# radhofan/Fairify

Hardware: AMD Instinct MI355X
Metric: % partitions verified + partitions/sec on AC suite at 1/2/4/8 MI355X (higher is better)
Workload: dtype fp32

## Files before the change

fairify_amd/csrc/symbolic.hip:

```cpp
#include <hip/hip_runtime.h>

#include <tuple>

#include "args.h"
#include "launch.h"

#define FA_SYM_MAXC 48

struct SymCfg {
  int nc;
  int cdim[FA_SYM_MAXC];
  unsigned long long fold;
  int w_lds[FA_MAX_LAYERS];
  int b_lds[FA_MAX_LAYERS];
  int lds_floats;
  int stage_off;
  int stage_floats;
};

using SymShapeAny = FaShapeAny;
template <int... D>
using SymShape = FaShape<D...>;

template <class S>
struct SymLay {
  __host__ __device__ static constexpr int tiles(int n) { return (n + 15) >> 4; }
  __host__ __device__ static constexpr int w(int l) {
    int off = 0;
    for (int i = 0; i < l; ++i) off += tiles(S::dim(i)) * tiles(S::dim(i + 1)) * 256;
    return off;
  }
  __host__ __device__ static constexpr int b(int l) {
    int off = w(S::L);
    for (int i = 0; i < l; ++i) off += S::dim(i + 1);
    return off;
  }
  __host__ __device__ static constexpr int noff(int l) {
    int off = 0;
    for (int i = 0; i < l; ++i) off += S::dim(i + 1);
    return off;
  }
  static constexpr int STAGE = (b(S::L) + 3) & ~3;
  static constexpr int LDS = STAGE + FA_SYM_MAXC;
};

struct SymBox {
  const BoundArgs* a;
  int node, v, n0;
  __device__ __forceinline__ float lo(int d) const {
    float x = a->lo[(size_t)node * n0 + d];
    if (a->V > 0)
      for (int k = 0; k < a->npa; ++k)
        if (a->pa_idx[k] == d) x = a->values[v * a->npa + k];
    return x;
  }
  __device__ __forceinline__ float hi(int d) const {
    float x = a->hi[(size_t)node * n0 + d];
    if (a->V > 0)
      for (int k = 0; k < a->npa; ++k)
        if (a->pa_idx[k] == d) x = a->values[v * a->npa + k];
    return x;
  }
};

__device__ __forceinline__ int fa_trot(int rho) { return rho >> 3; }

template <int NT, int PG = 1>
struct SymSlab {
  static constexpr int TS = 16 * NT + 4;
  static constexpr int TILE1 = 2 * 16 * TS;
  static constexpr int TILE = 2 * TILE1;
  static constexpr int BOX = 3 * FA_SYM_MAXC;
  static constexpr int BOXTAB = PG > 1 ? 2 * PG * 32 : 0;
  static constexpr int FLOATS = (TILE + 2 * PG * BOX + BOXTAB + 3) & ~3;
};

template <bool PAIR, int TM>
struct SymForm {
  static constexpr bool CR = !PAIR && TM >= 2;
};

__device__ __forceinline__ void fa_pq_to_ul(const f32x4& P, const f32x4& Q, int fc, float gg, f32x4& U,
                                            f32x4& L) {
  const float sl = (fc == 1 || fc == 3) ? 2.f * gg : 0.f;
#pragma unroll
  for (int i = 0; i < 4; ++i) {
    const float q = Q[i], e = sl * fabsf(q);
    U[i] = (P[i] + q) + e;
    L[i] = (P[i] - q) - e;
  }
}

template <int NT, bool PAIR, int PG = 1, bool CR = false, class S = SymShapeAny, bool MASK = true>
__device__ __forceinline__ bool fa_sym_epilogue(const NetDesc& net, const BoundArgs& a, const SymCfg& cfg,
                                                const float* smem, float* T, const float* bxv_in, const int* cdim_s,
                                                int l, int r_in, int node_in, int r2, int node2, bool v2, int lane,
                                                int jt0, const f32x4 (&U)[2][NT],
                                                const f32x4 (&Lq)[2][NT], float (&nu)[2][NT][4],
                                                float (&nlo)[2][NT][4]) {
  constexpr int TS = SymSlab<NT>::TS;
  constexpr bool CS = S::L > 0;
  constexpr bool CL = CS && PG == 1;
  const int col = lane & 15, grp = lane >> 4;
  const int n_out = CS ? S::dim(l + 1) : net.dims[l + 1];
  const float* sb = smem + (CL ? SymLay<S>::b(l) : cfg.b_lds[l]);
  const bool last = CS ? l == S::L - 1 : l == net.n_layers - 1;
  const float gg = net.g_gemm[l];
  const float gc = net.g_conc;
  const float gi = net.g_one;
  const float unit = net.unit;
  const float gnext = last ? 0.f : (CR ? net.g_fwd[l + 1] : net.g_gemm[l + 1]);
  const int noff = CL ? SymLay<S>::noff(l) : net.neuron_off[l];
  const int nc = cfg.nc;
  const int n0 = CS ? S::dim(0) : net.dims[0];
  const int tsub = lane >> 5;
  const bool second = PAIR && tsub;
  constexpr int PS = 16 / PG;
  const int gbox = PG > 1 ? col / PS : 0;
  const int bidx = tsub * PG + gbox;
  const int r = PG > 1 ? r_in + bidx : (second ? r2 : r_in);
  const int node = PG > 1 ? (a.V > 0 ? r / a.V : r) : (second ? node2 : node_in);
  const float* bxv = bxv_in + (PG > 1 ? bidx : (second ? 1 : 0)) * SymSlab<NT, PG>::BOX;
  const int jt = PAIR ? jt0 : jt0 + tsub;
  const int n_out_t = n_out;
  const bool nl_act = PG > 1 ? r < a.R : (16 * jt < n_out_t && (!second || v2));
  const int ob = (lane >> 4) & 1;
  float* Trow = T + tsub * SymSlab<NT>::TILE1 + (ob * 16 + col) * TS + fa_trot(ob * 16 + col);
#pragma unroll
    for (int u = 0; u < 2; ++u)
#pragma unroll
      for (int ct = 0; ct < NT; ++ct)
#pragma unroll
        for (int i = 0; i < 4; ++i) {
          const int ru = 4 * grp + i, rl = 16 + 4 * grp + i;
          T[u * SymSlab<NT>::TILE1 + ru * TS + fa_trot(ru) + ct * 16 + col] = U[u][ct][i];
          T[u * SymSlab<NT>::TILE1 + rl * TS + fa_trot(rl) + ct * 16 + col] = Lq[u][ct][i];
        }
    __builtin_amdgcn_wave_barrier();
    const int j = PG > 1 ? col - gbox * PS : 16 * jt + col;
    const bool jv = j < n_out;
    float v[16 * NT];
#pragma unroll
    for (int c = 0; c < 16 * NT; ++c) v[c] = Trow[c];
    const float braw = sb[PG > 1 ? col : min(j, n_out - 1)];
    const float b = jv ? braw : 0.f;
    float s1 = 0.f, s2 = 0.f, mg = 0.f;
#pragma unroll
    for (int c = 4; c < 16 * NT; ++c) {
      const float av = fabsf(v[c]);
      s1 = fmaf(v[c], bxv[c], s1);
      s2 = fmaf(av, bxv[FA_SYM_MAXC + c], s2);
      mg = fmaf(av, bxv[2 * FA_SYM_MAXC + c], mg);
    }
    float mn = s1 - s2, mx = s1 + s2;
    const float cr = v[0];
    float er = v[1], ivr = v[2], ier = v[3];
    const float sgn = ob ? -1.f : 1.f;
    er *= sgn;
    ier *= sgn;
    const float c0 = cr + b;
    const float mgc = mg;
    mn += c0; mx += c0; mg += fabsf(c0);
    const float iv = ivr + b;
    const float eI = ier * (1.f + 2.f * gg) + gg * fabsf(b);
    const float e = er * (1.f + 2.f * gg) + gg * fabsf(b);
    float bound;
    if (ob == 0) bound = fminf(iv + gi * fabsf(iv) + eI, mx + gc * mg + e);
    else bound = fmaxf(iv - gi * fabsf(iv) - eI, mn - gc * mg - e);
    const float other = __shfl_xor(bound, 16, 64);
    const float ub = ob == 0 ? bound : other;
    const float lb = ob == 0 ? other : bound;
    if (nl_act && jv && a.layer_lb) {
      if (ob == 0) a.layer_ub[(size_t)r * net.n_neurons + noff + j] = ub;
      else a.layer_lb[(size_t)r * net.n_neurons + noff + j] = lb;
    }
    if (last) {
      if (PG > 1) {
        if (nl_act && j == 0) {
          float* Cf = ob == 0 ? a.Uc : a.Lc;
          if (ob == 0) {
            a.out_ub[r] = ub; a.U0[r] = c0; a.Ue[r] = e;
          } else {
            a.out_lb[r] = lb; a.L0[r] = c0; a.Le[r] = e;
          }
          for (int d = 0; d < n0; ++d)
            if ((cfg.fold >> d) & 1ull) Cf[(size_t)r * n0 + d] = 0.f;
          for (int c = 0; c < nc; ++c) Cf[(size_t)r * n0 + cdim_s[c]] = Trow[4 + c];
        }
      } else if (nl_act && jt == 0) {
        if (col == 0) {
          if (ob == 0) {
            a.out_ub[r] = ub; a.U0[r] = c0; a.Ue[r] = e;
          } else {
            a.out_lb[r] = lb; a.L0[r] = c0; a.Le[r] = e;
          }
        }
        float* Cf = (ob == 0 ? a.Uc : a.Lc) + (size_t)r * n0;
        const float* row0 = T + tsub * SymSlab<NT>::TILE1 + (ob * 16) * TS + fa_trot(ob * 16) + 4;
        const unsigned long long fold = cfg.fold;
        for (int d = col; d < n0; d += 16) {
          const bool folded = (fold >> d) & 1ull;
          const int c = d - __popcll(fold & ((1ull << d) - 1ull));
          const float x = row0[folded ? 0 : c];
          Cf[d] = folded ? 0.f : x;
        }
      }
      return false;
    }
    bool forced = false, fact = false;
    if (MASK && nl_act && jv) {
      if (a.dead_in) forced = a.dead_in[(size_t)r * net.n_hidden + noff + j] != 0;
      else if (a.dead_part) forced = a.dead_part[(size_t)a.node_part[node] * net.n_hidden + noff + j] != 0;
      if (a.phase_in) {
        const int8_t ph = a.phase_in[(size_t)r * net.n_hidden + noff + j];
        forced = forced || ph < 0;
        fact = ph > 0;
        if (ob == 0 && a.infeas && ((ph < 0 && lb > 0.f) || (ph > 0 && ub < 0.f))) a.infeas[r] = 1;
      }
    }
    const bool isdead = ub <= 0.f;
    const bool isact = lb >= 0.f;
    if (MASK && nl_act && ob == 0 && jv && a.dead_out) a.dead_out[(size_t)r * net.n_hidden + noff + j] = isdead ? 1 : 0;
    const bool zero = isdead || forced || !jv;
    const float aa = mn - gc * mg + e;
    const float bb = mx + gc * mg + e;
    const bool chord = !zero && !isact && !fact && aa < 0.f;
    const float sc = (bb / (bb - aa)) * (1.f + 4.f * unit);
    const float shift = e - aa;
    const float cc = c0 * sc + sc * shift;
    const float sU = zero ? 0.f : (chord ? sc : 1.f);
    const float cU = zero ? 0.f : (chord ? cc : c0);
    const float mU = zero ? 0.f : (chord ? sc * mgc * (1.f + 8.f * unit) + fabsf(cc) : mg);
    const float eU = zero ? 0.f : (chord ? 4.f * unit * sc * (mg + fabsf(shift)) : e);
    const float aL = mn - gc * mg - e;
    const float bL = mx + gc * mg - e;
    const bool lam1 = !zero && (isact || ((bL > 0.f) && (bL > -aL)));
    const bool up = ob == 0;
    const float ivn = zero ? 0.f : fmaxf(up ? ub : lb, 0.f);
    const float s = up ? sU : (lam1 ? 1.f : 0.f);
    const float cnew = up ? cU : (lam1 ? c0 : 0.f);
    const float en = up ? eU : (lam1 ? e : 0.f);
    const float mgn = up ? mU : (lam1 ? mg : 0.f);
    const float mg_b = CR ? mgn + __shfl_xor(mgn, 16, 64) : mgn;
    const float iv_b = CR ? fmaxf(ivn, __shfl_xor(ivn, 16, 64)) : ivn;
    v[0] = cnew;
    v[1] = sgn * (en + gnext * mg_b);
    v[2] = ivn;
    v[3] = sgn * (gnext * iv_b);
#pragma unroll
    for (int c = 4; c < 16 * NT; ++c) v[c] *= s;
    if (nl_act) {
#pragma unroll
      for (int c = 0; c < 16 * NT; ++c) Trow[c] = v[c];
    }
    __builtin_amdgcn_wave_barrier();
#pragma unroll
    for (int u = 0; u < 2; ++u)
#pragma unroll
      for (int ct = 0; ct < NT; ++ct)
#pragma unroll
        for (int i = 0; i < 4; ++i) {
          const int ru = 4 * grp + i, rl = 16 + 4 * grp + i;
          const float xu = T[u * SymSlab<NT>::TILE1 + ru * TS + fa_trot(ru) + ct * 16 + col];
          const float xl = T[u * SymSlab<NT>::TILE1 + rl * TS + fa_trot(rl) + ct * 16 + col];
          nu[u][ct][i] = CR ? 0.5f * (xu + xl) : xu;
          nlo[u][ct][i] = CR ? 0.5f * (xu - xl) : xl;
        }
    __builtin_amdgcn_wave_barrier();
    return true;
}

template <int NT, int TM, bool PAIR, int PG = 1, class S = SymShapeAny, bool MASK = true>
__device__ __forceinline__ void fa_sym_layer(const NetDesc& net, const BoundArgs& a, const SymCfg& cfg,
                                             const float* smem, float* T, const float* bxv, const int* cdim_s,
                                             int l, int r, int node, int r2, int node2, bool v2, int lane,
                                             const float (&B)[NT][PAIR ? 2 : TM][2][4],
                                             float (&A)[NT][PAIR ? 2 : TM][2][4]) {
  constexpr int TMS = PAIR ? 2 : TM;
  constexpr bool CR = SymForm<PAIR, TM>::CR;
  constexpr int TS = SymSlab<NT>::TS;
  constexpr bool CS = S::L > 0;
  constexpr bool CL = CS && PG == 1;
  const int col = lane & 15, grp = lane >> 4;
  const int n_in = CS ? S::dim(l) : net.dims[l], n_out = CS ? S::dim(l + 1) : net.dims[l + 1];
  const int tin = (n_in + 15) >> 4, tout = (n_out + 15) >> 4;
  const float* sw = smem + (CL ? SymLay<S>::w(l) : cfg.w_lds[l]);
  const bool last = CS ? l == S::L - 1 : l == net.n_layers - 1;
  const float gg = net.g_gemm[l];
  const int nc = cfg.nc;
  const int n0 = CS ? S::dim(0) : net.dims[0];
#ifndef FA_SYM_TIMING_NO_EPILOGUE
  if (PG > 1 && l == 0) {
    const float* boxtab = bxv + 2 * PG * SymSlab<NT, PG>::BOX;
    const float g0 = net.g_gemm[0];
    const int n0v = n0;
    f32x4 U[2][NT], Lq[2][NT];
#pragma unroll
    for (int u = 0; u < 2; ++u) {
#pragma unroll
      for (int ct = 0; ct < NT; ++ct) U[u][ct] = Lq[u][ct] = f32x4{0.f, 0.f, 0.f, 0.f};
#pragma unroll
      for (int g = 0; g < PG; ++g) {
        const float* bt = boxtab + (u * PG + g) * 32;
        const float4 w4 = reinterpret_cast<const float4*>(sw)[g * 64 + lane];
        const float wv[4] = {w4.x, w4.y, w4.z, w4.w};
#pragma unroll
        for (int i = 0; i < 4; ++i) {
          const int k = 4 * grp + i;
          const bool kv = k < n0v;
          const float xl = kv ? bt[k] : 0.f, xh = kv ? bt[16 + k] : 0.f;
          const bool folded = kv && ((cfg.fold >> k) & 1ull);
          const float m = fmaxf(fabsf(xl), fabsf(xh));
          const float wp = fmaxf(wv[i], 0.f), wn = fminf(wv[i], 0.f);
#pragma unroll
          for (int ct = 0; ct < NT; ++ct) {
            const int c = ct * 16 + col;
            float vu = 0.f, vl = 0.f;
            if (kv) {
              if (c >= 4) {
                vu = vl = (!folded && c - 4 < nc && cdim_s[c - 4] == k) ? 1.f : 0.f;
              } else if (c == 0) {
                vu = vl = folded ? xl : 0.f;
              } else if (c == 1) {
                vu = g0 * m; vl = -vu;
              } else if (c == 2) {
                vu = xh; vl = xl;
              } else {
                vu = g0 * fabsf(xh); vl = -(g0 * fabsf(xl));
              }
            }
            U[u][ct] = fa_mfma4(wp, vu, U[u][ct]);
            Lq[u][ct] = fa_mfma4(wp, vl, Lq[u][ct]);
            U[u][ct] = fa_mfma4(wn, vl, U[u][ct]);
            Lq[u][ct] = fa_mfma4(wn, vu, Lq[u][ct]);
          }
        }
      }
    }
    float nu[2][NT][4], nlo[2][NT][4];
    if (!fa_sym_epilogue<NT, PAIR, PG, CR, S, MASK>(net, a, cfg, smem, T, bxv, cdim_s, l, r, node, r2, node2, v2, lane, 0, U, Lq,
                                       nu, nlo))
      return;
#pragma unroll
    for (int u = 0; u < 2; ++u)
#pragma unroll
      for (int ct = 0; ct < NT; ++ct)
#pragma unroll
        for (int i = 0; i < 4; ++i) {
          A[ct][u][0][i] = nu[u][ct][i];
          A[ct][u][1][i] = nlo[u][ct][i];
        }
    return;
  }
  if (PG == 1 && last && n_out == 1) {
    constexpr int NB = PAIR ? 2 : 1;
    float su[NB][NT], sl[NB][NT];
#pragma unroll
    for (int bi = 0; bi < NB; ++bi)
#pragma unroll
      for (int ct = 0; ct < NT; ++ct) su[bi][ct] = sl[bi][ct] = 0.f;
#pragma unroll
    for (int t = 0; t < TM; ++t) {
      if (t >= tin) break;
      const float4 w4 = reinterpret_cast<const float4*>(sw)[t * 64 + grp * 16];
      const float wv[4] = {w4.x, w4.y, w4.z, w4.w};
#pragma unroll
      for (int i = 0; i < 4; ++i) {
        const float wp = fmaxf(wv[i], 0.f), wn = fminf(wv[i], 0.f);
#pragma unroll
        for (int bi = 0; bi < NB; ++bi)
#pragma unroll
          for (int ct = 0; ct < NT; ++ct) {
            const int bt = PAIR ? bi : t;
            if (CR) {
              su[bi][ct] = fmaf(wv[i], B[ct][bt][0][i], su[bi][ct]);
              sl[bi][ct] = fmaf(fabsf(wv[i]), B[ct][bt][1][i], sl[bi][ct]);
            } else {
              su[bi][ct] = fmaf(wp, B[ct][bt][0][i], fmaf(wn, B[ct][bt][1][i], su[bi][ct]));
              sl[bi][ct] = fmaf(wp, B[ct][bt][1][i], fmaf(wn, B[ct][bt][0][i], sl[bi][ct]));
            }
          }
      }
    }
    f32x4 U[2][NT], Lq[2][NT];
#pragma unroll
    for (int ct = 0; ct < NT; ++ct) U[1][ct] = Lq[1][ct] = f32x4{0.f, 0.f, 0.f, 0.f};
#pragma unroll
    for (int bi = 0; bi < NB; ++bi)
#pragma unroll
      for (int ct = 0; ct < NT; ++ct) {
        float xu = su[bi][ct], xl = sl[bi][ct];
        xu += __shfl_xor(xu, 16, 64);
        xl += __shfl_xor(xl, 16, 64);
        xu += __shfl_xor(xu, 32, 64);
        xl += __shfl_xor(xl, 32, 64);
        U[bi][ct] = f32x4{grp == 0 ? xu : 0.f, 0.f, 0.f, 0.f};
        Lq[bi][ct] = f32x4{grp == 0 ? xl : 0.f, 0.f, 0.f, 0.f};
        if (CR) fa_pq_to_ul(f32x4(U[bi][ct]), f32x4(Lq[bi][ct]), ct * 16 + col, gg, U[bi][ct], Lq[bi][ct]);
      }
    float nu[2][NT][4], nlo[2][NT][4];
    fa_sym_epilogue<NT, PAIR, PG, CR, S, MASK>(net, a, cfg, smem, T, bxv, cdim_s, l, r, node, r2, node2, v2, lane, 0, U, Lq,
                                  nu, nlo);
    return;
  }
#endif
#pragma unroll
  for (int jt0 = 0; jt0 < TM; jt0 += 2) {
    if (jt0 >= tout) break;
    f32x4 U[2][NT], Lq[2][NT];
#pragma unroll
    for (int u = 0; u < 2; ++u) {
      const int jt = jt0 + u;
#pragma unroll
      for (int ct = 0; ct < NT; ++ct) {
        U[u][ct] = f32x4{0.f, 0.f, 0.f, 0.f};
        Lq[u][ct] = f32x4{0.f, 0.f, 0.f, 0.f};
      }
      if (PAIR ? (jt0 > 0) : (jt >= tout || jt >= TM)) continue;
      const float4* wq = reinterpret_cast<const float4*>(sw) + (size_t)(PAIR ? 0 : jt) * tin * 64 + lane;
#pragma unroll
      for (int t = 0; t < TM; ++t) {
        if (t >= tin) break;
        const float4 w4 = wq[t * 64];
        const float wv[4] = {w4.x, w4.y, w4.z, w4.w};
#pragma unroll
        for (int i = 0; i < 4; ++i) {
          const float wp = fmaxf(wv[i], 0.f), wn = fminf(wv[i], 0.f);
#pragma unroll
          for (int ct = 0; ct < NT; ++ct) {
            const int bt = PAIR ? u : t;
            const float bu = B[ct][bt][0][i], bl = B[ct][bt][1][i];
            if (CR) {
              U[u][ct] = fa_mfma4(wv[i], bu, U[u][ct]);
              Lq[u][ct] = fa_mfma4(fabsf(wv[i]), bl, Lq[u][ct]);
            } else {
              U[u][ct] = fa_mfma4(wp, bu, U[u][ct]);
              Lq[u][ct] = fa_mfma4(wp, bl, Lq[u][ct]);
              U[u][ct] = fa_mfma4(wn, bl, U[u][ct]);
              Lq[u][ct] = fa_mfma4(wn, bu, Lq[u][ct]);
            }
          }
        }
      }
      if (CR) {
#pragma unroll
        for (int ct = 0; ct < NT; ++ct)
          fa_pq_to_ul(f32x4(U[u][ct]), f32x4(Lq[u][ct]), ct * 16 + col, gg, U[u][ct], Lq[u][ct]);
      }
    }
    float nu[2][NT][4], nlo[2][NT][4];
#ifdef FA_SYM_TIMING_NO_EPILOGUE
#pragma unroll
    for (int u = 0; u < 2; ++u)
#pragma unroll
      for (int ct = 0; ct < NT; ++ct)
#pragma unroll
        for (int i = 0; i < 4; ++i) {
          nu[u][ct][i] = U[u][ct][i] * 1e-3f;
          nlo[u][ct][i] = Lq[u][ct][i] * 1e-3f;
        }
    if (l == net.n_layers - 1) {
      if (lane == 0) a.out_lb[r] = nu[0][0][0] + nlo[0][0][1];
      continue;
    }
#else
    if (!fa_sym_epilogue<NT, PAIR, PG, CR, S, MASK>(net, a, cfg, smem, T, bxv, cdim_s, l, r, node, r2, node2, v2, lane, jt0, U,
                                       Lq, nu, nlo))
      continue;
#endif
#pragma unroll
    for (int u = 0; u < 2; ++u) {
      if (jt0 + u >= TMS) break;
#pragma unroll
      for (int ct = 0; ct < NT; ++ct)
#pragma unroll
        for (int i = 0; i < 4; ++i) {
          A[ct][jt0 + u][0][i] = nu[u][ct][i];
          A[ct][jt0 + u][1][i] = nlo[u][ct][i];
        }
    }
  }
}

#ifndef FA_SYM_WPE7
#define FA_SYM_WPE7 2
#endif
#ifndef FA_SYM_WPE4
#define FA_SYM_WPE4 2
#endif
#define FA_SYM_WAVES_PER_EU(NT, TM, PAIR) \
  ((PAIR) ? 3 : ((TM) == 2 ? 3 : ((TM) == 4 ? FA_SYM_WPE4 : ((TM) == 7 ? FA_SYM_WPE7 : 1))))

template <int NT, int TM, bool PAIR, int PG, class S, bool MASK, int... LS>
__device__ __forceinline__ void fa_sym_layers_c(std::integer_sequence<int, LS...>, const NetDesc& net,
                                                const BoundArgs& a, const SymCfg& cfg, const float* smem, float* T,
                                                const float* bxv, const int* cdim_s, int r, int node, int r2,
                                                int node2, bool v2, int lane, float (&XA)[NT][PAIR ? 2 : TM][2][4],
                                                float (&XB)[NT][PAIR ? 2 : TM][2][4]) {
  ((LS & 1 ? fa_sym_layer<NT, TM, PAIR, PG, S, MASK>(net, a, cfg, smem, T, bxv, cdim_s, LS, r, node, r2, node2, v2,
                                                     lane, XB, XA)
           : fa_sym_layer<NT, TM, PAIR, PG, S, MASK>(net, a, cfg, smem, T, bxv, cdim_s, LS, r, node, r2, node2, v2,
                                                     lane, XA, XB)),
   ...);
}

#ifndef FA_SYM_BIG_THREADS
#define FA_SYM_BIG_THREADS 512
#endif
#define FA_SYM_THREADS(TM) ((TM) == 7 ? FA_SYM_BIG_THREADS : FA_THREADS)

#ifndef FA_SYM_PREFETCH
#define FA_SYM_PREFETCH 1
#endif

template <int NT, int TM, bool PAIR, class S>
struct SymTune {
  static constexpr int THREADS = FA_SYM_THREADS(TM);
  static constexpr int WPE = FA_SYM_WAVES_PER_EU(NT, TM, PAIR);
};
#define FA_SYM_TUNE(NT, TM, THREADS_, WPE_, ...)            \
  template <>                                                \
  struct SymTune<NT, TM, false, FaShape<__VA_ARGS__>> {      \
    static constexpr int THREADS = THREADS_;                 \
    static constexpr int WPE = WPE_;                         \
  };
FA_SYM_TUNE(1, 7, 256, 3, 13, 100, 1)

__device__ __forceinline__ void fa_sym_box_values(float l0, float h0, float* bv, int lane) {
  float mid = 0.5f * (l0 + h0), rad = 0.5f * (h0 - l0), mm = fmaxf(fabsf(l0), fabsf(h0));
  const bool lattice = l0 == rintf(l0) && h0 == rintf(h0) && fabsf(l0) < 4194304.f && fabsf(h0) < 4194304.f;
  if (!lattice) {
    rad = nextafterf(fmaxf(h0 - mid, mid - l0), INFINITY);
    mm = nextafterf(fabsf(mid) + rad, INFINITY);
  }
  bv[lane] = mid;
  bv[FA_SYM_MAXC + lane] = rad;
  bv[2 * FA_SYM_MAXC + lane] = mm;
}

template <int NT, bool CR, int TMS>
__device__ __forceinline__ void fa_sym_operand0(float xl, float xh, bool kv, bool folded, int k, float g0,
                                                const int (&role)[NT], const int (&cdm)[NT],
                                                float (&XA)[NT][TMS][2][4], int t, int i) {
  const float m = fmaxf(fabsf(xl), fabsf(xh));
#pragma unroll
  for (int ct = 0; ct < NT; ++ct) {
    float vu = 0.f, vl = 0.f;
    if (kv) {
      switch (role[ct]) {
        case 0: vu = (!folded && cdm[ct] == k) ? 1.f : 0.f; vl = CR ? 0.f : vu; break;
        case 1: vu = folded ? xl : 0.f; vl = CR ? 0.f : vu; break;
        case 2: vu = CR ? 0.f : g0 * m; vl = CR ? g0 * m : -vu; break;
        case 3:
          vu = CR ? 0.5f * (xh + xl) : xh;
          vl = CR ? 0.5f * (xh - xl) : xl;
          break;
        case 4:
          vu = CR ? 0.5f * g0 * (fabsf(xh) - fabsf(xl)) : g0 * fabsf(xh);
          vl = CR ? 0.5f * g0 * (fabsf(xh) + fabsf(xl)) : -(g0 * fabsf(xl));
          break;
        default: break;
      }
    }
    XA[ct][t][0][i] = vu;
    XA[ct][t][1][i] = vl;
  }
}

template <int NT, int TM, bool PAIR, int PG, class S, bool MASK>
__device__ __forceinline__ void fa_sym_rows(const NetDesc& net, const BoundArgs& a, const SymCfg& cfg, float* smem,
                                            const int* cdim_s, int lds_floats) {
  constexpr int THREADS = SymTune<NT, TM, PAIR, S>::THREADS;
  constexpr bool CR = SymForm<PAIR, TM>::CR;
  constexpr int TMS = PAIR ? 2 : TM;
  const int tid = threadIdx.x;
  const int lane = tid & 63;
  const int grp = lane >> 4;
  const int wave = tid >> 6;
  const int nw = THREADS / 64;
  const int n0 = S::L > 0 ? S::dim(0) : net.dims[0];
  const int nc = cfg.nc;
  const float g0 = net.g_gemm[0];
  float* T = smem + lds_floats + wave * SymSlab<NT, PG>::FLOATS;
  float* bxv = T + SymSlab<NT>::TILE;
  const int tin0 = (n0 + 15) >> 4;
  int role[NT], cdm[NT];
#pragma unroll
  for (int ct = 0; ct < NT; ++ct) {
    const int c = ct * 16 + (lane & 15);
    role[ct] = c == 0 ? 1 : c == 1 ? 2 : c == 2 ? 3 : c == 3 ? 4 : (c - 4 < nc ? 0 : 5);
    cdm[ct] = (role[ct] == 0) ? cdim_s[c - 4] : -1;
  }
  constexpr int RPW = PAIR ? 2 * PG : 1;
  if constexpr (!PAIR && S::L > 0 && FA_SYM_PREFETCH) {
    float* btab = bxv + SymSlab<NT>::BOX;
    static_assert(SymSlab<NT>::BOX >= 128, "box table in the second box's slot");
    static_assert(S::dim(0) <= 64, "lane d carries input dim d");
    const int V = a.V, R = a.R;
    int pslot = -1;
    if (V > 0)
      for (int k = 0; k < a.npa; ++k)
        if (a.pa_idx[k] == lane) pslot = k;
    const int dl = min(lane, n0 - 1);
    const int stride = gridDim.x * nw;
    const bool filt = a.skip_status != nullptr;
    auto node_of = [&](int rr) { return V > 0 ? rr / V : rr; };
    auto fetch = [&](int rr, int node, float& blo, float& bhi) {
      blo = a.lo[(size_t)node * n0 + dl];
      bhi = a.hi[(size_t)node * n0 + dl];
      if (pslot >= 0) blo = bhi = a.values[(rr - node * V) * a.npa + pslot];
    };
    int r = __builtin_amdgcn_readfirstlane(blockIdx.x * nw + wave);
    float blo = 0.f, bhi = 0.f;
    int st = 3, part1 = 0;
    int node = 0;
    if (r < R) {
      node = node_of(r);
      fetch(r, node, blo, bhi);
      if (filt) st = a.skip_status[a.skip_part[node]];
      if (filt && r + stride < R) part1 = a.skip_part[node_of(r + stride)];
    }
    for (; r < R; r += stride) {
      const int rn = r + stride;
      float nlo = 0.f, nhi = 0.f;
      int nst = 3, part2 = 0, nnode = 0;
      if (rn < R) {
        nnode = node_of(rn);
        fetch(rn, nnode, nlo, nhi);
        if (filt) nst = a.skip_status[part1];
        if (filt && rn + stride < R) part2 = a.skip_part[node_of(rn + stride)];
      }
      if (st == 3 || st == 4) {
        btab[lane] = blo;
        btab[64 + lane] = bhi;
        __builtin_amdgcn_wave_barrier();
        if (lane < FA_SYM_MAXC) {
          const int d = (lane >= 4 && lane - 4 < nc) ? cdim_s[lane - 4] : -1;
          fa_sym_box_values(d >= 0 ? btab[max(d, 0)] : 0.f, d >= 0 ? btab[64 + max(d, 0)] : 0.f, bxv, lane);
        }
        float XA[NT][TMS][2][4], XB[NT][TMS][2][4];
#pragma unroll
        for (int t = 0; t < TMS; ++t) {
          if (t >= tin0) break;
          const float4 l4 = reinterpret_cast<const float4*>(btab)[(4 * t + grp) & 15];
          const float4 h4 = reinterpret_cast<const float4*>(btab + 64)[(4 * t + grp) & 15];
          const float xl4[4] = {l4.x, l4.y, l4.z, l4.w}, xh4[4] = {h4.x, h4.y, h4.z, h4.w};
#pragma unroll
          for (int i = 0; i < 4; ++i) {
            const int k = 16 * t + 4 * grp + i;
            const bool kv = k < n0;
            const float xl = kv ? xl4[i] : 0.f, xh = kv ? xh4[i] : 0.f;
            fa_sym_operand0<NT, CR>(xl, xh, kv, kv && ((cfg.fold >> k) & 1ull), k, g0, role, cdm, XA, t, i);
          }
        }
        __builtin_amdgcn_wave_barrier();
        fa_sym_layers_c<NT, TM, PAIR, PG, S, MASK>(std::make_integer_sequence<int, S::L>{}, net, a, cfg, smem, T, bxv,
                                                   cdim_s, r, node, r, node, false, lane, XA, XB);
        __builtin_amdgcn_wave_barrier();
      }
      blo = nlo;
      bhi = nhi;
      st = nst;
      part1 = part2;
      node = nnode;
    }
    return;
  }
  for (int r0 = (blockIdx.x * nw + wave) * RPW; r0 < a.R; r0 += gridDim.x * nw * RPW) {
    const int r = __builtin_amdgcn_readfirstlane(r0);
    const bool v2 = PAIR && r + 1 < a.R;
    const int rb = v2 ? r + 1 : r;
    if (a.skip_status) {
      bool any = false;
#pragma unroll
      for (int bi = 0; bi < RPW; ++bi) {
        const int rr = min(r + bi, a.R - 1);
        const int8_t s1 = a.skip_status[a.skip_part[a.V > 0 ? rr / a.V : rr]];
        any = any || s1 == 3 || s1 == 4;
      }
      if (!any) continue;
    }
    SymBox bxs[RPW];
#pragma unroll
    for (int bi = 0; bi < RPW; ++bi) {
      SymBox& bx = bxs[bi];
      const int rr = PG > 1 ? min(r + bi, a.R - 1) : (bi ? rb : r);
      bx.a = &a;
      bx.n0 = n0;
      bx.node = a.V > 0 ? rr / a.V : rr;
      bx.v = a.V > 0 ? rr - bx.node * a.V : 0;
      if (lane < FA_SYM_MAXC) {
        float* bv = bxv + bi * SymSlab<NT>::BOX;
        const int d = (lane >= 4 && lane - 4 < nc) ? cdim_s[lane - 4] : -1;
        fa_sym_box_values(d >= 0 ? bx.lo(d) : 0.f, d >= 0 ? bx.hi(d) : 0.f, bv, lane);
      }
      if (PG > 1 && lane < 32) {
        const int d = lane & 15;
        float* bt = bxv + 2 * PG * SymSlab<NT, PG>::BOX + bi * 32;
        bt[lane] = d < n0 ? (lane < 16 ? bx.lo(d) : bx.hi(d)) : 0.f;
      }
    }
    const SymBox& bx = bxs[0];
    float XA[NT][TMS][2][4], XB[NT][TMS][2][4];
#pragma unroll
    for (int t = 0; t < TMS; ++t) {
      if (PG > 1) break;
      if (!PAIR && t >= tin0) break;
      const SymBox& bt = bxs[PAIR ? t : 0];
#pragma unroll
      for (int i = 0; i < 4; ++i) {
        const int k = (PAIR ? 0 : 16 * t) + 4 * grp + i;
        float xl = 0.f, xh = 0.f;
        const bool kv = k < n0;
        if (kv) {
          xl = bt.lo(k);
          xh = bt.hi(k);
        }
        fa_sym_operand0<NT, CR>(xl, xh, kv, kv && ((cfg.fold >> k) & 1ull), k, g0, role, cdm, XA, t, i);
      }
    }
    __builtin_amdgcn_wave_barrier();
    if constexpr (S::L > 0) {
      fa_sym_layers_c<NT, TM, PAIR, PG, S, MASK>(std::make_integer_sequence<int, S::L>{}, net, a, cfg, smem, T, bxv,
                                                 cdim_s, r, bx.node, rb, bxs[RPW - 1].node, v2, lane, XA, XB);
    } else {
      for (int l = 0; l < net.n_layers; ++l) {
        if (l & 1)
          fa_sym_layer<NT, TM, PAIR, PG, S, MASK>(net, a, cfg, smem, T, bxv, cdim_s, l, r, bx.node, rb,
                                                  bxs[RPW - 1].node, v2, lane, XB, XA);
        else
          fa_sym_layer<NT, TM, PAIR, PG, S, MASK>(net, a, cfg, smem, T, bxv, cdim_s, l, r, bx.node, rb,
                                                  bxs[RPW - 1].node, v2, lane, XA, XB);
      }
    }
    __builtin_amdgcn_wave_barrier();
  }
}

template <int NT, int TM, bool PAIR, int PG = 1, class S = SymShapeAny>
__global__ void __launch_bounds__((SymTune<NT, TM, PAIR, S>::THREADS))
    __attribute__((amdgpu_waves_per_eu(SymTune<NT, TM, PAIR, S>::WPE))) fa_sym_kernel(NetDesc net, BoundArgs a, SymCfg cfg) {
  constexpr int THREADS = SymTune<NT, TM, PAIR, S>::THREADS;
  constexpr bool CL = S::L > 0 && PG == 1;
  extern __shared__ __attribute__((aligned(16))) float smem[];
  const int tid = threadIdx.x;
  const int stage_floats = CL ? SymLay<S>::STAGE : cfg.stage_floats;
  const int lds_floats = CL ? SymLay<S>::LDS : cfg.lds_floats;
  {
    const float4* src = reinterpret_cast<const float4*>(a.flat + cfg.stage_off);
    float4* dst = reinterpret_cast<float4*>(smem);
    for (int e = tid; e < (stage_floats >> 2); e += THREADS) dst[e] = src[e];
  }
  int* cdim_s = reinterpret_cast<int*>(smem + lds_floats - FA_SYM_MAXC);
  for (int c = tid; c < FA_SYM_MAXC; c += THREADS) cdim_s[c] = c < cfg.nc ? cfg.cdim[c] : -1;
  __syncthreads();
  constexpr bool LEAN = S::L > 0 && !PAIR;
  const bool masked = !LEAN || a.dead_in || a.dead_part || a.phase_in || a.dead_out;
  if (masked) fa_sym_rows<NT, TM, PAIR, PG, S, true>(net, a, cfg, smem, cdim_s, lds_floats);
  else fa_sym_rows<NT, TM, PAIR, PG, S, !LEAN>(net, a, cfg, smem, cdim_s, lds_floats);
}


namespace {

typedef void (*SymKernel)(NetDesc, BoundArgs, SymCfg);

template <int NT, int TM, bool PAIR = false, int PG = 1>
SymKernel sym_ptr() {
  return fa_sym_kernel<NT, TM, PAIR, PG>;
}

bool use_pack() {
  static const bool v = [] {
    const char* e = getenv("FAIRIFY_SYM_PACK");
    return !(e && *e == '0');
  }();
  return v;
}

SymKernel select_packed(int pg) {
  switch (pg) {
    case 2: return sym_ptr<1, 1, true, 2>();
    case 4: return sym_ptr<1, 1, true, 4>();
    default: return nullptr;
  }
}

bool use_pair() {
  static const bool v = [] {
    const char* e = getenv("FAIRIFY_SYM_PAIR");
    return !(e && *e == '0');
  }();
  return v;
}

int max_tm() {
  static const int v = [] {
    const char* e = getenv("FAIRIFY_SYM_MAX_TM");
    return (e && *e) ? atoi(e) : 10;
  }();
  return v;
}

#define FA_SYM_GRID(X) X(1, 1) X(1, 2) X(1, 4) X(1, 7) X(1, 10) X(2, 1) X(2, 2) X(2, 4) X(2, 10) X(3, 1) X(3, 2)

int tm_bucket(int NT, int TM) {
  if (TM > max_tm()) return 0;
  const int b = fa_tm_bucket(TM);
  if (NT == 2 && b == 7) return 10;
  if (NT == 3 && b > 2) return 0;
  return NT >= 1 && NT <= 3 ? b : 0;
}

SymKernel select_kernel(int NT, int tmb) {
  if (NT == 1 && tmb == 1 && use_pair()) return sym_ptr<1, 1, true>();
  switch (16 * NT + tmb) {
#define FA_SYM_CASE(NT_, TM_) \
  case 16 * NT_ + TM_: return sym_ptr<NT_, TM_>();
    FA_SYM_GRID(FA_SYM_CASE)
#undef FA_SYM_CASE
    default: return nullptr;
  }
}

#define FA_SYM_SHAPES(X)                                                                              \
  X(1, 4, false, 1, 13, 64, 32, 16, 8, 4, 1)                \
  X(2, 4, false, 1, 13, 64, 32, 16, 8, 4, 1)          \
  X(2, 4, false, 1, 16, 64, 32, 16, 8, 4, 1)                                                \
  X(1, 4, false, 1, 13, 64, 64, 1)                                                          \
  X(1, 4, false, 1, 13, 50, 1)                                                              \
  X(1, 7, false, 1, 13, 100, 100, 1)                                                        \
  X(1, 7, false, 1, 13, 100, 1)                                                             \
               \
  X(1, 1, true, 1, 13, 16, 8, 1)                                                            \
  X(1, 1, true, 1, 13, 12, 12, 1)                                                           \
  X(1, 1, true, 1, 13, 10, 10, 10, 10, 1)                                                  \
                                                         \
  X(1, 1, true, 2, 13, 5, 5, 1)                                                             \
  X(1, 1, true, 2, 13, 5, 5, 5, 5, 1)

constexpr int sym_key(int nt, int tm, bool pair, int pg) { return ((16 * nt + tm) * 2 + (pair ? 1 : 0)) * 8 + pg; }

typedef bool (*SymLayoutOk)(const NetDesc&, const SymCfg&);
struct SymInst {
  SymKernel k = nullptr;
  SymLayoutOk ok = nullptr;
  int threads = 0, wpe = 0;
  SymInst(std::nullptr_t = nullptr) {}
  SymInst(SymKernel k_, SymLayoutOk ok_, int threads_, int wpe_) : k(k_), ok(ok_), threads(threads_), wpe(wpe_) {}
};
template <class S>
bool sym_layout_ok(const NetDesc& net, const SymCfg& cfg);
template <int NT, int TM, bool PAIR, int PG, class S>
SymInst sym_inst() {
  typedef SymTune<NT, TM, PAIR, S> Tune;
  return SymInst(fa_sym_kernel<NT, TM, PAIR, PG, S>, sym_layout_ok<S>, Tune::THREADS, Tune::WPE);
}
template <class S>
bool sym_layout_ok(const NetDesc& net, const SymCfg& cfg) {
  for (int l = 0; l < S::L; ++l)
    if (cfg.w_lds[l] != SymLay<S>::w(l) || cfg.b_lds[l] != SymLay<S>::b(l) || net.neuron_off[l] != SymLay<S>::noff(l))
      return false;
  return cfg.stage_floats == SymLay<S>::STAGE && cfg.lds_floats == SymLay<S>::LDS;
}

struct SymPick {
  SymKernel k;
  int NT, tmb;
  bool pair;
  int pg;
  bool shaped;
  int threads, wpe;
  int err;
};

SymPick pick_sym(const NetDesc& net, unsigned long long fold_mask, SymCfg& cfg) {
  SymPick p{};
  const int n0 = net.dims[0];
  if (n0 > 64) return p;
  cfg.fold = fold_mask;
  int nc = 0;
  for (int d = 0; d < n0; ++d)
    if (!((fold_mask >> d) & 1ull)) {
      if (nc >= FA_SYM_MAXC) return p;
      cfg.cdim[nc++] = d;
    }
  cfg.nc = nc;
  if (n0 < 64 && (fold_mask >> n0)) return p;
  if (nc != n0 - __builtin_popcountll(fold_mask)) return p;
  for (int c = 1; c < nc; ++c)
    if (cfg.cdim[c] <= cfg.cdim[c - 1]) return p;
  const int cols = nc + 4;
  p.NT = (cols + 15) / 16;
  p.tmb = tm_bucket(p.NT, fa_widest_tiles(net, 0, net.n_layers));
  SymKernel k = select_kernel(p.NT, p.tmb);
  if (!k) return p;
  p.pair = k == sym_ptr<1, 1, true>();
  p.pg = (p.pair && net.pack_g > 1 && net.dims[0] <= 16 && use_pack()) ? net.pack_g : 1;
  if (p.pg > 1) k = select_packed(p.pg);
  if (!k) return p;
  int off = 0;
  if (p.pg > 1) {
    cfg.w_lds[0] = 0;
    off = p.pg * 256;
    for (int l = 1; l < net.n_layers; ++l) {
      cfg.w_lds[l] = off;
      off += 256;
    }
    for (int l = 0; l < net.n_layers; ++l) {
      cfg.b_lds[l] = off;
      off += 16;
    }
    if (off != net.pack_floats) p.err = -1;
    cfg.stage_off = net.pack_off;
  } else {
    off = fa_lay_weights(net, net.n_layers, cfg.w_lds, 0);
    off = fa_lay_biases(net, net.n_layers, cfg.b_lds, off);
    off = ((off + 3) & ~3);
    if (off != net.wperm_floats) p.err = -1;
    cfg.stage_off = net.wperm_off;
  }
  cfg.stage_floats = off;
  cfg.lds_floats = off + FA_SYM_MAXC;
  p.threads = FA_SYM_THREADS(p.pair ? 1 : p.tmb);
  p.wpe = FA_SYM_WAVES_PER_EU(p.NT, p.tmb, p.pair);
  if (!fa_env_off("FAIRIFY_SYM_SHAPED")) {
#define FA_SYM_ENTRY(NT, TM, PAIR, PG, ...) \
  {sym_key(NT, TM, PAIR, PG),                \
   {__VA_ARGS__},                            \
   sym_inst<NT, TM, PAIR, PG, SymShape<__VA_ARGS__>>()},
    static const std::vector<FaShaped<SymInst>> v = {FA_SYM_SHAPES(FA_SYM_ENTRY)};
#undef FA_SYM_ENTRY
    const SymInst si = fa_find_shaped(v, net, sym_key(p.NT, p.tmb, p.pair, p.pg));
    if (si.k && !p.err && (p.pg > 1 || si.ok(net, cfg))) {
      k = si.k;
      p.shaped = true;
      p.threads = si.threads;
      p.wpe = si.wpe;
    }
  }
  p.k = k;
  return p;
}

struct SymGeom {
  int threads, rows_per_block;
  size_t bytes;
};
SymGeom sym_geom(const SymPick& p, const SymCfg& cfg) {
  int slab = 0;
  switch (p.NT) {
    case 1:
      slab = p.pg == 2 ? SymSlab<1, 2>::FLOATS : p.pg == 4 ? SymSlab<1, 4>::FLOATS : SymSlab<1>::FLOATS;
      break;
    case 2: slab = SymSlab<2>::FLOATS; break;
    default: slab = SymSlab<3>::FLOATS; break;
  }
  SymGeom g;
  g.threads = p.threads;
  g.rows_per_block = (g.threads / 64) * (p.pair ? 2 * p.pg : 1);
  g.bytes = (size_t)(cfg.lds_floats + (g.threads / 64) * slab) * sizeof(float);
  return g;
}

}

extern "C" int fa_sym_shaped(const NetDesc& net, unsigned long long fold_mask) {
  SymCfg cfg{};
  return pick_sym(net, fold_mask, cfg).shaped;
}

extern "C" int fa_sym_try_launch(const NetDesc& net, BoundArgs a, unsigned long long fold_mask,
                                 hipStream_t stream) {
  if (!a.symbolic || a.R <= 0) return 0;
  SymCfg cfg{};
  const SymPick p = pick_sym(net, fold_mask, cfg);
  const SymKernel k = p.k;
  if (!k) return 0;
  if (p.err) return p.err;
  const SymGeom g = sym_geom(p, cfg);
  if (g.bytes > 160 * 1024) return 0;
  const int per_cu = fa_blocks_per_cu((const void*)k, g.threads, g.bytes);
  if (!per_cu) return -4;
  long long blocks = (a.R + g.rows_per_block - 1) / g.rows_per_block;
  const long long cap = (long long)fa_device_cus() * per_cu;
  if (blocks > cap) blocks = cap;
  hipLaunchKernelGGL(k, dim3((unsigned)blocks), dim3(g.threads), g.bytes, stream, net, a, cfg);
  const hipError_t e = hipGetLastError();
  return e == hipSuccess ? 1 : -(int)e;
}

extern "C" int fa_sym_geometry(const NetDesc& net, unsigned long long fold_mask, int* out) {
  SymCfg cfg{};
  const SymPick p = pick_sym(net, fold_mask, cfg);
  if (!p.k || p.err) return 0;
  const SymGeom g = sym_geom(p, cfg);
  if (g.bytes > 160 * 1024) return 0;
  const int per_cu = fa_blocks_per_cu((const void*)p.k, g.threads, g.bytes);
  if (!per_cu) return 0;
  out[0] = g.threads;
  out[1] = (int)g.bytes;
  out[2] = per_cu;
  out[3] = fa_device_cus();
  out[4] = g.rows_per_block;
  out[5] = p.wpe;
  out[6] = p.shaped;
  hipFuncAttributes fa{};
  out[7] = hipFuncGetAttributes(&fa, (const void*)p.k) == hipSuccess ? fa.numRegs : 0;
  return 1;
}

#define FA_SYM_LDS(NT, TM) FA_LDS_K((sym_ptr<NT, TM>())),
#define FA_SYM_SHAPE_LDS(NT, TM, PAIR, PG, ...) FA_LDS_K((fa_sym_kernel<NT, TM, PAIR, PG, SymShape<__VA_ARGS__>>)),
FA_LDS_REGISTER(FA_SYM_GRID(FA_SYM_LDS) FA_LDS_K((sym_ptr<1, 1, true>())), FA_LDS_K((sym_ptr<1, 1, true, 2>())),
                FA_LDS_K((sym_ptr<1, 1, true, 4>())));
FA_LDS_REGISTER(FA_SYM_SHAPES(FA_SYM_SHAPE_LDS));
#undef FA_SYM_LDS
#undef FA_SYM_SHAPE_LDS
```

Measured before the change: 299,300.

## Add prefetching row loop and lean path for shaped narrow paired symbolic kernels

```diff
diff --git a/fairify_amd/csrc/symbolic.hip b/fairify_amd/csrc/symbolic.hip
--- a/fairify_amd/csrc/symbolic.hip
+++ b/fairify_amd/csrc/symbolic.hip
@@ -22,15 +22,17 @@
 template <int... D>
 using SymShape = FaShape<D...>;
 
-template <class S>
+template <class S, int PG = 1>
 struct SymLay {
   __host__ __device__ static constexpr int tiles(int n) { return (n + 15) >> 4; }
   __host__ __device__ static constexpr int w(int l) {
+    if (PG > 1) return l == 0 ? 0 : PG * 256 + (l - 1) * 256;
     int off = 0;
     for (int i = 0; i < l; ++i) off += tiles(S::dim(i)) * tiles(S::dim(i + 1)) * 256;
     return off;
   }
   __host__ __device__ static constexpr int b(int l) {
+    if (PG > 1) return PG * 256 + (S::L - 1) * 256 + 16 * l;
     int off = w(S::L);
     for (int i = 0; i < l; ++i) off += S::dim(i + 1);
     return off;
@@ -100,17 +102,17 @@
                                                 float (&nlo)[2][NT][4]) {
   constexpr int TS = SymSlab<NT>::TS;
   constexpr bool CS = S::L > 0;
-  constexpr bool CL = CS && PG == 1;
+  constexpr bool CL = CS;
   const int col = lane & 15, grp = lane >> 4;
   const int n_out = CS ? S::dim(l + 1) : net.dims[l + 1];
-  const float* sb = smem + (CL ? SymLay<S>::b(l) : cfg.b_lds[l]);
+  const float* sb = smem + (CL ? SymLay<S, PG>::b(l) : cfg.b_lds[l]);
   const bool last = CS ? l == S::L - 1 : l == net.n_layers - 1;
   const float gg = net.g_gemm[l];
   const float gc = net.g_conc;
   const float gi = net.g_one;
   const float unit = net.unit;
   const float gnext = last ? 0.f : (CR ? net.g_fwd[l + 1] : net.g_gemm[l + 1]);
-  const int noff = CL ? SymLay<S>::noff(l) : net.neuron_off[l];
+  const int noff = CL ? SymLay<S, PG>::noff(l) : net.neuron_off[l];
   const int nc = cfg.nc;
   const int n0 = CS ? S::dim(0) : net.dims[0];
   const int tsub = lane >> 5;
@@ -175,7 +177,27 @@
       else a.layer_lb[(size_t)r * net.n_neurons + noff + j] = lb;
     }
     if (last) {
-      if (PG > 1) {
+      if (PG > 1 && CS) {
+        if (nl_act) {
+          if (j == 0) {
+            if (ob == 0) {
+              a.out_ub[r] = ub; a.U0[r] = c0; a.Ue[r] = e;
+            } else {
+              a.out_lb[r] = lb; a.L0[r] = c0; a.Le[r] = e;
+            }
+          }
+          float* Cf = (ob == 0 ? a.Uc : a.Lc) + (size_t)r * n0;
+          const int rho = ob * 16 + gbox * PS;
+          const float* row0 = T + tsub * SymSlab<NT>::TILE1 + rho * TS + fa_trot(rho) + 4;
+          const unsigned long long fold = cfg.fold;
+          for (int d = j; d < n0; d += PS) {
+            const bool folded = (fold >> d) & 1ull;
+            const int c = d - __popcll(fold & ((1ull << d) - 1ull));
+            const float x = row0[folded ? 0 : c];
+            Cf[d] = folded ? 0.f : x;
+          }
+        }
+      } else if (PG > 1) {
         if (nl_act && j == 0) {
           float* Cf = ob == 0 ? a.Uc : a.Lc;
           if (ob == 0) {
@@ -280,11 +302,11 @@
   constexpr bool CR = SymForm<PAIR, TM>::CR;
   constexpr int TS = SymSlab<NT>::TS;
   constexpr bool CS = S::L > 0;
-  constexpr bool CL = CS && PG == 1;
+  constexpr bool CL = CS;
   const int col = lane & 15, grp = lane >> 4;
   const int n_in = CS ? S::dim(l) : net.dims[l], n_out = CS ? S::dim(l + 1) : net.dims[l + 1];
   const int tin = (n_in + 15) >> 4, tout = (n_out + 15) >> 4;
-  const float* sw = smem + (CL ? SymLay<S>::w(l) : cfg.w_lds[l]);
+  const float* sw = smem + (CL ? SymLay<S, PG>::w(l) : cfg.w_lds[l]);
   const bool last = CS ? l == S::L - 1 : l == net.n_layers - 1;
   const float gg = net.g_gemm[l];
   const int nc = cfg.nc;
@@ -512,19 +534,30 @@
 #ifndef FA_SYM_PREFETCH
 #define FA_SYM_PREFETCH 1
 #endif
+#ifndef FA_SYM_PREFETCH_NARROW
+#define FA_SYM_PREFETCH_NARROW 1
+#endif
+#ifndef FA_SYM_LEAN_NARROW
+#define FA_SYM_LEAN_NARROW 1
+#endif
 
 template <int NT, int TM, bool PAIR, class S>
 struct SymTune {
   static constexpr int THREADS = FA_SYM_THREADS(TM);
   static constexpr int WPE = FA_SYM_WAVES_PER_EU(NT, TM, PAIR);
+  static constexpr bool PREFETCH = PAIR ? FA_SYM_PREFETCH_NARROW != 0 : FA_SYM_PREFETCH != 0;
+  static constexpr bool LEAN = !PAIR || FA_SYM_LEAN_NARROW != 0;
 };
-#define FA_SYM_TUNE(NT, TM, THREADS_, WPE_, ...)            \
-  template <>                                                \
-  struct SymTune<NT, TM, false, FaShape<__VA_ARGS__>> {      \
-    static constexpr int THREADS = THREADS_;                 \
-    static constexpr int WPE = WPE_;                         \
+#define FA_SYM_TUNE(NT, TM, PAIR, THREADS_, WPE_, PREFETCH_, LEAN_, ...) \
+  template <>                                                             \
+  struct SymTune<NT, TM, PAIR, FaShape<__VA_ARGS__>> {                    \
+    static constexpr int THREADS = THREADS_;                              \
+    static constexpr int WPE = WPE_;                                      \
+    static constexpr bool PREFETCH = PREFETCH_;                           \
+    static constexpr bool LEAN = LEAN_;                                   \
   };
-FA_SYM_TUNE(1, 7, 256, 3, 13, 100, 1)
+FA_SYM_TUNE(1, 7, false, 256, 3, FA_SYM_PREFETCH != 0, true, 13, 100, 1)
+FA_SYM_TUNE(1, 1, true, FA_THREADS, 4, FA_SYM_PREFETCH_NARROW != 0, FA_SYM_LEAN_NARROW != 0, 13, 12, 12, 1)
 
 __device__ __forceinline__ void fa_sym_box_values(float l0, float h0, float* bv, int lane) {
   float mid = 0.5f * (l0 + h0), rad = 0.5f * (h0 - l0), mm = fmaxf(fabsf(l0), fabsf(h0));
@@ -592,7 +625,7 @@
     cdm[ct] = (role[ct] == 0) ? cdim_s[c - 4] : -1;
   }
   constexpr int RPW = PAIR ? 2 * PG : 1;
-  if constexpr (!PAIR && S::L > 0 && FA_SYM_PREFETCH) {
+  if constexpr (!PAIR && S::L > 0 && SymTune<NT, TM, PAIR, S>::PREFETCH) {
     float* btab = bxv + SymSlab<NT>::BOX;
     static_assert(SymSlab<NT>::BOX >= 128, "box table in the second box's slot");
     static_assert(S::dim(0) <= 64, "lane d carries input dim d");
@@ -666,6 +699,95 @@
     }
     return;
   }
+  if constexpr (PAIR && S::L > 0 && SymTune<NT, TM, PAIR, S>::PREFETCH) {
+    static_assert(NT == 1 && S::dim(0) <= 16 && RPW <= 4, "lane 16 b + d carries input dim d of box b");
+    constexpr int BOX = SymSlab<NT, PG>::BOX;
+    const int V = a.V, R = a.R;
+    const int d = lane & 15, bl = min(grp, RPW - 1);
+    const bool owner = lane < 16 * RPW;
+    float* btab = PG > 1 ? bxv + 2 * PG * BOX + bl * 32 : bxv + bl * BOX + 16;
+    int pslot = -1;
+    if (V > 0)
+      for (int k = 0; k < a.npa; ++k)
+        if (a.pa_idx[k] == d) pslot = k;
+    const int dl = min(d, n0 - 1);
+    const int stride = gridDim.x * nw * RPW;
+    const bool filt = a.skip_status != nullptr;
+    auto row_of = [&](int r0) { return min(r0 + bl, R - 1); };
+    auto node_of = [&](int rr) { return V > 0 ? rr / V : rr; };
+    auto fetch = [&](int rr, int node, float& blo, float& bhi) {
+      blo = a.lo[(size_t)node * n0 + dl];
+      bhi = a.hi[(size_t)node * n0 + dl];
+      if (pslot >= 0) blo = bhi = a.values[(rr - node * V) * a.npa + pslot];
+    };
+    int r = __builtin_amdgcn_readfirstlane((blockIdx.x * nw + wave) * RPW);
+    float blo = 0.f, bhi = 0.f;
+    int st = 3, part1 = 0, node1 = 0;
+    if (r < R) {
+      const int rr = row_of(r), node = node_of(rr);
+      fetch(rr, node, blo, bhi);
+      if (filt) st = a.skip_status[a.skip_part[node]];
+      if (r + stride < R) {
+        node1 = node_of(row_of(r + stride));
+        if (filt) part1 = a.skip_part[node1];
+      }
+    }
+    for (; r < R; r += stride) {
+      const int rn = r + stride;
+      float nlo = 0.f, nhi = 0.f;
+      int nst = 3, part2 = 0, node2 = 0;
+      if (rn < R) {
+        fetch(row_of(rn), node1, nlo, nhi);
+        if (filt) nst = a.skip_status[part1];
+        if (rn + stride < R) {
+          node2 = node_of(row_of(rn + stride));
+          if (filt) part2 = a.skip_part[node2];
+        }
+      }
+      if (__ballot(st == 3 || st == 4) != 0) {
+        const bool v2 = r + 1 < R;
+        const int rb = v2 ? r + 1 : r;
+        if (owner) {
+          btab[d] = d < n0 ? blo : 0.f;
+          btab[16 + d] = d < n0 ? bhi : 0.f;
+        }
+        __builtin_amdgcn_wave_barrier();
+        if (owner) {
+          const int dc = (d >= 4 && d - 4 < nc) ? cdim_s[d - 4] : -1;
+          fa_sym_box_values(dc >= 0 ? btab[max(dc, 0)] : 0.f, dc >= 0 ? btab[16 + max(dc, 0)] : 0.f, bxv + bl * BOX, d);
+        }
+        float XA[NT][TMS][2][4], XB[NT][TMS][2][4];
+        if constexpr (PG == 1) {
+#pragma unroll
+          for (int t = 0; t < 2; ++t) {
+            const float* bt = bxv + t * BOX + 16;
+            const float4 l4 = reinterpret_cast<const float4*>(bt)[grp];
+            const float4 h4 = reinterpret_cast<const float4*>(bt + 16)[grp];
+            const float xl4[4] = {l4.x, l4.y, l4.z, l4.w}, xh4[4] = {h4.x, h4.y, h4.z, h4.w};
+#pragma unroll
+            for (int i = 0; i < 4; ++i) {
+              const int k = 4 * grp + i;
+              const bool kv = k < n0;
+              const float xl = kv ? xl4[i] : 0.f, xh = kv ? xh4[i] : 0.f;
+              fa_sym_operand0<NT, CR>(xl, xh, kv, kv && ((cfg.fold >> k) & 1ull), k, g0, role, cdm, XA, t, i);
+            }
+          }
+        }
+        __builtin_amdgcn_wave_barrier();
+        const int node_a = MASK ? node_of(r) : 0;
+        const int node_b = MASK ? node_of(PG > 1 ? min(r + RPW - 1, R - 1) : rb) : 0;
+        fa_sym_layers_c<NT, TM, PAIR, PG, S, MASK>(std::make_integer_sequence<int, S::L>{}, net, a, cfg, smem, T, bxv,
+                                                   cdim_s, r, node_a, rb, node_b, v2, lane, XA, XB);
+        __builtin_amdgcn_wave_barrier();
+      }
+      blo = nlo;
+      bhi = nhi;
+      st = nst;
+      part1 = part2;
+      node1 = node2;
+    }
+    return;
+  }
   for (int r0 = (blockIdx.x * nw + wave) * RPW; r0 < a.R; r0 += gridDim.x * nw * RPW) {
     const int r = __builtin_amdgcn_readfirstlane(r0);
     const bool v2 = PAIR && r + 1 < a.R;
@@ -741,11 +863,11 @@
 __global__ void __launch_bounds__((SymTune<NT, TM, PAIR, S>::THREADS))
     __attribute__((amdgpu_waves_per_eu(SymTune<NT, TM, PAIR, S>::WPE))) fa_sym_kernel(NetDesc net, BoundArgs a, SymCfg cfg) {
   constexpr int THREADS = SymTune<NT, TM, PAIR, S>::THREADS;
-  constexpr bool CL = S::L > 0 && PG == 1;
+  constexpr bool CL = S::L > 0;
   extern __shared__ __attribute__((aligned(16))) float smem[];
   const int tid = threadIdx.x;
-  const int stage_floats = CL ? SymLay<S>::STAGE : cfg.stage_floats;
-  const int lds_floats = CL ? SymLay<S>::LDS : cfg.lds_floats;
+  const int stage_floats = CL ? SymLay<S, PG>::STAGE : cfg.stage_floats;
+  const int lds_floats = CL ? SymLay<S, PG>::LDS : cfg.lds_floats;
   {
     const float4* src = reinterpret_cast<const float4*>(a.flat + cfg.stage_off);
     float4* dst = reinterpret_cast<float4*>(smem);
@@ -754,7 +876,7 @@
   int* cdim_s = reinterpret_cast<int*>(smem + lds_floats - FA_SYM_MAXC);
   for (int c = tid; c < FA_SYM_MAXC; c += THREADS) cdim_s[c] = c < cfg.nc ? cfg.cdim[c] : -1;
   __syncthreads();
-  constexpr bool LEAN = S::L > 0 && !PAIR;
+  constexpr bool LEAN = S::L > 0 && SymTune<NT, TM, PAIR, S>::LEAN;
   const bool masked = !LEAN || a.dead_in || a.dead_part || a.phase_in || a.dead_out;
   if (masked) fa_sym_rows<NT, TM, PAIR, PG, S, true>(net, a, cfg, smem, cdim_s, lds_floats);
   else fa_sym_rows<NT, TM, PAIR, PG, S, !LEAN>(net, a, cfg, smem, cdim_s, lds_floats);
@@ -849,19 +971,19 @@
   SymInst(std::nullptr_t = nullptr) {}
   SymInst(SymKernel k_, SymLayoutOk ok_, int threads_, int wpe_) : k(k_), ok(ok_), threads(threads_), wpe(wpe_) {}
 };
-template <class S>
+template <class S, int PG>
 bool sym_layout_ok(const NetDesc& net, const SymCfg& cfg);
 template <int NT, int TM, bool PAIR, int PG, class S>
 SymInst sym_inst() {
   typedef SymTune<NT, TM, PAIR, S> Tune;
-  return SymInst(fa_sym_kernel<NT, TM, PAIR, PG, S>, sym_layout_ok<S>, Tune::THREADS, Tune::WPE);
-}
-template <class S>
+  return SymInst(fa_sym_kernel<NT, TM, PAIR, PG, S>, sym_layout_ok<S, PG>, Tune::THREADS, Tune::WPE);
+}
+template <class S, int PG>
 bool sym_layout_ok(const NetDesc& net, const SymCfg& cfg) {
+  typedef SymLay<S, PG> Lay;
   for (int l = 0; l < S::L; ++l)
-    if (cfg.w_lds[l] != SymLay<S>::w(l) || cfg.b_lds[l] != SymLay<S>::b(l) || net.neuron_off[l] != SymLay<S>::noff(l))
-      return false;
-  return cfg.stage_floats == SymLay<S>::STAGE && cfg.lds_floats == SymLay<S>::LDS;
+    if (cfg.w_lds[l] != Lay::w(l) || cfg.b_lds[l] != Lay::b(l) || net.neuron_off[l] != Lay::noff(l)) return false;
+  return cfg.stage_floats == Lay::STAGE && cfg.lds_floats == Lay::LDS;
 }
 
 struct SymPick {
@@ -932,7 +1054,7 @@
     static const std::vector<FaShaped<SymInst>> v = {FA_SYM_SHAPES(FA_SYM_ENTRY)};
 #undef FA_SYM_ENTRY
     const SymInst si = fa_find_shaped(v, net, sym_key(p.NT, p.tmb, p.pair, p.pg));
-    if (si.k && !p.err && (p.pg > 1 || si.ok(net, cfg))) {
+    if (si.k && !p.err && si.ok(net, cfg)) {
       k = si.k;
       p.shaped = true;
       p.threads = si.threads;
```

Result: slower. 295,500 (-1.3%).
